# GoogleCloudPlatform/plspm-python

Measured on AMD Instinct MI355X. Metric: bootstrap replicates/sec (6-LV satisfaction model, N=10k), higher is better.
Workload: dtype f64

## Files before the change

plspm-python_amd/csrc/kernels_gram_i8.h:

```cpp
#pragma once
#include <type_traits>
#include "wave_ops.h"

typedef int i32x4 __attribute__((ext_vector_type(4)));
#define I8_SLACK_KB 6
#ifndef I8_DEFAULT_VAR
#define I8_DEFAULT_VAR 3
#endif

__global__ void __launch_bounds__(256) zs_max_kernel(const double* __restrict__ Xa, long N, int PA, int C, const int* __restrict__ pair_p, const int* __restrict__ pair_q,
                                                      int npair, int RB, unsigned long long* __restrict__ pair_max) {
    extern __shared__ __attribute__((aligned(16))) unsigned char smem_raw[];
    double* tile = reinterpret_cast<double*>(smem_raw);
    const int pitch = C | 1;
    const long r0 = (long)blockIdx.x * RB;
    const int nr = (int)min((long)RB, N - r0);
    for (int e = threadIdx.x; e < RB * C; e += 256) {
        const int r = e / C, c = e - r * C;
        tile[r * pitch + c] = (r < nr) ? Xa[(r0 + r) * PA + c] : 0.0;
    }
    __syncthreads();
    for (int j = threadIdx.x; j < npair; j += 256) {
        const int p = pair_p[j], q = pair_q[j];
        double mx = 0.0;
// ... 84 lines not shown
#pragma unroll
            for (int s = 0; s < S; ++s) {
                const int d = (int)((v + 128) & 255) - 128;
                v = (v - d) >> 8;
                dig[s][t] = (unsigned char)(d & 255);
            }
        }
    }
#pragma unroll
    for (int s = 0; s < S; ++s) {
        uint4 w;
        unsigned u[4];
#pragma unroll
        for (int c = 0; c < 4; ++c) u[c] = (unsigned)dig[s][4 * c] | ((unsigned)dig[s][4 * c + 1] << 8) | ((unsigned)dig[s][4 * c + 2] << 16) | ((unsigned)dig[s][4 * c + 3] << 24);
        w.x = u[0]; w.y = u[1]; w.z = u[2]; w.w = u[3];
        if (shape == 16) Zs[((long)kb * NT + (long)pgw * S + s) * 64 + sub * 16 + r] = w;
        else Zs[((long)kb * NT + ((long)pgw * S + s) * 2 + (sub >> 1)) * 64 + (sub & 1) * 32 + r] = w;
    }
}

#define I8_HIST_KB 1024
#define I8_HIST_KB_BYTES 2048
template <bool BYTES>
__global__ void __launch_bounds__(1024) resample_i8_kernel(int N, int KB, int MT, int shape, const int* __restrict__ idx, uint64_t seed, int64_t rep0, uint4* __restrict__ Cd,
                                                           int* __restrict__ err) {
    extern __shared__ __attribute__((aligned(16))) unsigned char smem_raw[];
    unsigned* hist = reinterpret_cast<unsigned*>(smem_raw);
    const int tid = threadIdx.x, nthr = blockDim.x;
    const long b = blockIdx.x;
    constexpr int WKB = BYTES ? I8_HIST_KB_BYTES : I8_HIST_KB;
    const int kb0 = (int)blockIdx.y * WKB, KBw = min(WKB, KB - kb0);
    const unsigned r0 = (unsigned)kb0 * 64u, rspan = (unsigned)KBw * 64u;
    const int nwords = KBw * (BYTES ? 16 : 32);
    auto count = [&](unsigned w) {
        if (BYTES) atomicAdd(&hist[w >> 2], 1u << (8u * (w & 3u)));
        else atomicAdd(&hist[w >> 1], (w & 1u) ? 0x10000u : 1u);
    };
    for (int i = tid; i < nwords; i += nthr) hist[i] = 0u;
    __syncthreads();
    if (idx) {
        const int* my = idx + b * (long)N;
        for (int i = tid; i < N; i += nthr) {
            const int r = my[i];
            if ((unsigned)r < (unsigned)N) { const unsigned w = (unsigned)r - r0; if (w < rspan) count(w); }
            else if (blockIdx.y == 0) atomicOr(err, 1);
        }
    } else {
        const uint64_t rep = (uint64_t)(rep0 + b);
        const int nq = (N + 3) >> 2;
        for (int q = tid; q < nq; q += nthr) {
            const u32x4 u = resample_quad(seed, rep, (uint32_t)q);
#pragma unroll
            for (int j = 0; j < 4; ++j)
                if (4 * q + j < N) { const unsigned w = to_index(u.v[j], (uint32_t)N) - r0; if (w < rspan) count(w); }
        }
    }
    __syncthreads();
    const int mt = (int)(b >> 4), r = (int)(b & 15);
    const uint4* h4 = reinterpret_cast<const uint4*>(hist);
    bool over = false;
    for (int c = tid; c < KBw * 4; c += nthr) {
        uint4 out;
        if (BYTES) {
            out = h4[c];
            over |= ((out.x | out.y | out.z | out.w) & 0x80808080u) != 0u;
        } else {
            const uint4 lo = h4[2 * c], hi = h4[2 * c + 1];
            const unsigned w[8] = {lo.x, lo.y, lo.z, lo.w, hi.x, hi.y, hi.z, hi.w};
            unsigned o[4];
#pragma unroll
            for (int k = 0; k < 4; ++k) {
                const unsigned a = w[2 * k], bb = w[2 * k + 1];
                over |= ((a | bb) & 0xff80ff80u) != 0u;
                o[k] = (a & 0xffu) | ((a >> 8) & 0xff00u) | ((bb & 0xffu) << 16) | ((bb << 8) & 0xff000000u);
            }
            out.x = o[0]; out.y = o[1]; out.z = o[2]; out.w = o[3];
        }
        const int kb = kb0 + (c >> 2), g = c & 3;
        if (shape == 16) Cd[((long)kb * MT + mt) * 64 + g * 16 + r] = out;
        else Cd[((long)kb * MT + (b >> 5) * 2 + (g >> 1)) * 64 + (g & 1) * 32 + (int)(b & 31)] = out;
    }
    if (over) atomicOr(err, 2);
}

#define I8_HIST_KB_NIB 4096
__device__ __forceinline__ unsigned nib_spread16(unsigned t) {
    t = (t | (t << 8)) & 0x00ff00ffu;
    return (t | (t << 4)) & 0x0f0f0f0fu;
}
__global__ void __launch_bounds__(1024) resample_i8_nib_kernel(int N, int KB, int MT, uint64_t seed, int64_t rep0, uint4* __restrict__ Cd, int* __restrict__ err, int force_slow) {
    extern __shared__ __attribute__((aligned(16))) unsigned char smem_raw[];
    unsigned* hist = reinterpret_cast<unsigned*>(smem_raw);
    __shared__ unsigned tot[2];
    const int tid = threadIdx.x, nthr = blockDim.x;
    const long b = blockIdx.x;
    const int kb0 = (int)blockIdx.y * I8_HIST_KB_NIB, KBw = min(I8_HIST_KB_NIB, KB - kb0);
    const unsigned r0 = (unsigned)kb0 * 64u, rspan = (unsigned)KBw * 64u;
    const int nwords = KBw * 8;
    const uint64_t rep = (uint64_t)(rep0 + b);
    const int nq = (N + 3) >> 2;
    const int mt = (int)(b >> 4), r = (int)(b & 15);
    for (int i = tid; i < nwords; i += nthr) hist[i] = 0u;
    if (tid < 2) tot[tid] = 0u;
// ... 560 lines not shown
```

plspm-python_amd/csrc/kernels_gram_i8p.h:

```cpp
#pragma once
#include <type_traits>

template <int S, int MW, int SCHED = 0>
struct GramI8PStep {
    static constexpr int NW = 4, NB = 2 * S, NMFMA = MW * NB;
    static constexpr int PERB = (NB + NW - 1) / NW;
    struct Tab { int a[8], d[8], r[16]; bool ok; };
    static constexpr Tab build() {
        Tab t{};
        if (SCHED == 0) {
            for (int i = 0; i < MW; ++i) t.a[i] = i == 0 ? 1 : NB * i + 1;
            for (int i = 0; i < PERB; ++i) t.d[i] = (i * NMFMA) / PERB + 4;
            for (int r = 0; r < NB; ++r) t.r[r] = (r * (NMFMA - 16)) / NB + 2;
            t.ok = true;
        } else if (SCHED == 2) {
            const int V = MW + PERB;
            bool used[128] = {};
            int na = 0, nd = 0;
            for (int k = 0; k < V; ++k) {
                int m = 1 + (k * NMFMA) / V;
                const bool a_ok = na < MW && m >= (na == 0 ? 1 : NB * na + 1);
                if (a_ok) t.a[na++] = m;
                else if (nd < PERB) t.d[nd++] = m;
                else { m = NB * na + 1; while (used[m]) ++m; t.a[na++] = m; }
// ... 35 lines not shown
    static_assert(MW * NB * 4 <= 240, "accumulator tiles must fit the AGPR half");
};

template <int S, int MTW, int VAR = 0>
struct GramI8P {
    static constexpr int NW = 4, NB = 2 * S, RT = NW * MTW;
    static constexpr int PERB = (NB + NW - 1) / NW;
    static constexpr bool BREG = ((VAR >> 4) & 1) != 0;
    static constexpr int SCHED = (VAR >> 5) & 3;
    static constexpr bool PAIRB = ((VAR >> 7) & 1) != 0 && !BREG;
    static constexpr int STAGE_BYTES = NB * 1024, NS = BREG ? 2 : PAIRB ? 5 : 3, AHEAD = BREG ? 2 : PAIRB ? 4 : 3;
    static constexpr size_t LDS_BYTES = (size_t)NS * STAGE_BYTES;
    static constexpr int RTS = RT - NW;
    static constexpr int ABL = VAR & 15;
};

template <int S, int MTW, int VAR = 0, bool SHORTS = false>
__global__ void __launch_bounds__(256) __attribute__((amdgpu_waves_per_eu(1, 1)))
gram_i8p_kernel(const uint4* __restrict__ Cd, const uint4* __restrict__ Zs, int KB, int MT, int NT, int ntx, int nty, const int* __restrict__ pair_dst,
                const double* __restrict__ pair_scale, int npair, long nrep, double* __restrict__ gram, long psize, int nty_short) {
    using G = GramI8P<S, MTW, VAR>;
    constexpr int NB = G::NB, RT = G::RT;
    extern __shared__ __attribute__((aligned(1024))) unsigned char smem_raw[];
    const int tid = threadIdx.x, lane = tid & 63;
    const int wave = __builtin_amdgcn_readfirstlane(tid >> 6);
    const int w = blockIdx.x;
    int slot = w >> 3, rows = nty, rbase = 0;
    bool shortT = false;
    if constexpr (SHORTS) {
        const int ntall = nty - nty_short, tper = (ntx * ntall + 7) >> 3;
        if (slot >= tper) { slot -= tper; rows = nty_short; rbase = ntall; shortT = true; }
        else rows = ntall;
    }
    const int total = ntx * rows, per = (total + 7) >> 3;
    const int gidx = (w & 7) * per + slot;
    if (slot >= per || gidx >= total) return;
    const int srow = 4 * ntx;
    const int sr = __builtin_amdgcn_readfirstlane(gidx / srow), rem = gidx - sr * srow;
    const int nr = min(4, rows - 4 * sr);
    const int tx = __builtin_amdgcn_readfirstlane(rem / nr), tyl = 4 * sr + (rem - tx * nr);
    const int ct0 = shortT ? rbase * RT + tyl * G::RTS : tyl * RT;

    const unsigned lds0 = (unsigned)(size_t)((__attribute__((address_space(3))) unsigned char*)smem_raw);
    const unsigned voff = (unsigned)lane * 16u;
    const long binc = (long)NT * 1024, ainc = (long)MT * 1024;

// ... 388 lines not shown
```

plspm-python_amd/csrc/model.h:

```cpp
#pragma once
#include <hip/hip_runtime.h>

#include <cstdint>
#include <string>
#include <utility>
#include <vector>

#include "../../include/plspm_hip_test.h"

inline thread_local std::string g_create_error;

hipError_t plspm_dmalloc(void** p, size_t bytes);
void plspm_dfree(void* p);
hipError_t plspm_hmalloc(void** p, size_t bytes);
void plspm_hfree(void* p);
hipError_t plspm_stream_acquire(hipStream_t* s);
void plspm_stream_release(hipStream_t s);

struct PermSpec;
struct StratSpec;
struct CvSpec;
struct JackSpec;

struct ProfSlot { std::vector<std::pair<hipEvent_t, hipEvent_t>> ev, pool; double total_ms = 0.0; int64_t launches = 0; };

struct plspm_model {
    int device = 0;
    hipStream_t stream = nullptr;
    bool owns_stream = true;
    int P = 0, L = 0, PA = 0, T = 0, scheme = 0, scaled = 1, max_iter = 100, kmax = 0, n_eff = 0, n_chol = 0;
    double tol = 1e-6;
// ... 34 lines not shown
    Buf gram2;
    plspm_model* stage2 = nullptr;
    plspm_model* stage1 = nullptr;
    std::vector<int> lv_first, col2_lv1, col2_p1, hcol, hidx;
    std::vector<int> lv_cols;
    int* d_lv_cols = nullptr;
    int *d_lv_first = nullptr, *d_col2_lv1 = nullptr, *d_col2_p1 = nullptr, *d_hcol = nullptr, *d_hidx = nullptr;
    Buf pseudo;
    Buf dcnt, ctable, Xt;
    long dcnt_stride = 0;
    bool Xt_valid = false, dcnt_ready = false;
    int nmx_K = 0, nmx_raw = 0;
    double *d_Xk = nullptr, *d_Mk = nullptr;
    int* d_rowid = nullptr;
    int* h_flag = nullptr;
    hipEvent_t ev_flag = nullptr;
    void* h_stage = nullptr;
    size_t h_stage_cap = 0;
    Buf scores;
    Buf xa, up_raw, up_ci, up_partial;
    int64_t rows_B = 0;
    bool err_clean = false;
    struct Tune { int wide_nw = 4, fit_chunks = 0, conv_pass = 0, conv_gy = 0, nm_threads = 0, solver_threads = 128, scores_tile = 0, gram_lds_kb = 0;
                  int gram_path = 0, i8_slices = 0, i8_min_batch = 1, i8_waves = 8, i8_rt = 0, i8_short = -1, i8_cus = 0, upload_direct = 0, i8_dma = 0, i8_variant = -1, solver_rows = 1, solver_wave = 1, solver_quad = 1, nm_counts8 = 1, nm_fast_lds = 1, nm_k16 = 1, nm_codes = 1, i8_ind = 1, i8_shape = 16, resample_aux = 0, i8_sched = 0, i8_priv = 1, boot_chunks = 0, boot_ratio = 60, boot_align = 0, i8_persist = 0, i8_min_slices = 0, i8_nostore = 0, nm_wave = 1, nm_live = 1, nm_mfma = 1, nm_direct16 = 1, i8_nibbles = 1, nm_wave16 = 1, nm_verify_rows = 0, nm_bound_shift = 0, wide_ring = 4, nm_subset = 4, nm_cat_one = 1, nm_cpl = 0, nm_c10 = 1, nm_vlong = 1, strat_rows = 0, boot_pass = 0; } tune;
    Buf zs, cd, cd1, err2, pair_tab, pair_scale, zs_stat, codes, ind8, tab8, scl8, pp_ctl;
    Buf sk_partial, sk_flags;
    unsigned sk_epoch = 0;
    int cu_count = 0;
    hipStream_t aux = nullptr;
    hipEvent_t ev_counts[2] = {nullptr, nullptr}, ev_cdfree[2] = {nullptr, nullptr};
    bool cdfree_set[2] = {false, false};
    int cd_slot = 0;
    bool zs_valid = false;
    bool zs_stats_ready = false;
    int zs_stats_S = 0;
    void* h_zstat = nullptr;
    size_t h_zstat_cap = 0;
    hipEvent_t ev_zstat = nullptr;
    int zs_S = 0, zs_KB = 0, zs_NT = 0, zs_npair = 0, zs_npg = 0;
    int zs_floor = 0;
    bool zs_ind = false;
    double zs_ratio = 0.0;
    Buf perm_thr, perm_member, perm_io;
    Buf strat_rows, strat_draws, strat_io, strat_u;
    std::vector<uint8_t> strat_member;
    Buf cv_fold, cv_thr, cv_idx, cv_off, cv_mom, cv_coef, cv_io, cv_pred, cv_tab;
    int64_t cv_reps = 0; int cv_k = 0;
    Buf jack_rows, jack_status, jack_iters, jack_io;
    int64_t jack_G = 0;
    bool assess_on = false;
    Buf assess_rows, assess_fit;
    int64_t assess_B = 0;
    bool micom_on = false;
    Buf micom_rows, micom_pool, micom_io;
    int64_t micom_B = 0;
// ... 126 lines not shown
```

plspm-python_amd/csrc/plspm_gram_i8.hip:

```cpp
#include "host_internal.h"

#include "philox.h"
#include "wave_ops.h"
#include "kernels_gram_i8.h"
#include "kernels_gram_i8p.h"

static constexpr size_t kZsBudget = (size_t)24 << 30;
static int cu_count_of(plspm_model* m) {
    if (!m->cu_count) {
        int n = 0;
        if (hipDeviceGetAttribute(&n, hipDeviceAttributeMultiprocessorCount, m->device) == hipSuccess) m->cu_count = n;
    }
    return m->cu_count;
}

bool nm_counts8_possible(const plspm_model* m) {
    return m->nonmetric && m->tune.nm_counts8 != 0 && m->tune.resample_aux == 0 && !m->aux && m->tune.i8_shape == 16 && m->nmx_K == 0 &&
           nm_dense_lds(plan_shape(m), m->tune.conv_pass, nullptr) != 0 && (!m->stage2 || nm_dense_lds(plan_shape(m->stage2), m->stage2->tune.conv_pass, nullptr) != 0);
}
bool gram_i8_closed(const plspm_model* m, int slices) {
    if (m->stage1 || m->N >= (1 << 24) || m->N < 2) return true;
    if (m->nonmetric && m->N > 65535 && !nm_counts8_possible(m)) return true;
    const size_t zs_bytes = (size_t)(i8_kblocks(m->N) + I8_SLACK_KB) * (size_t)(((i8_pairs(m) + 31) / 32) * 2 * (slices ? slices : 7)) * 1024;
    return zs_bytes > kZsBudget;
}
int choose_gram_path(const plspm_model* m, int64_t B) {
    if (m->tune.gram_path == 1 || gram_i8_closed(m, m->tune.i8_slices)) return 1;
    return (m->tune.gram_path == 2 || B >= m->tune.i8_min_batch) ? 2 : 1;
}

static int choose_slices(plspm_model* m, const unsigned long long* h, long npair, int* S_out, int floor) {
    double worst = 1e300;
    unsigned long long any = 0ull;
    for (long j = 0; j < npair; ++j) any |= h[2 * npair + j];
    for (long j = 0; j < npair; ++j) {
        const unsigned long long mb = h[j];
        if (mb == 0) continue;
        const int ef = (int)((mb >> 52) & 0x7ffull);
        if (ef < 64 || ef >= 0x7ff) { worst = 0.0; break; }
        double zmax;
        memcpy(&zmax, &mb, sizeof(double));
// ... 184 lines not shown
        if (!priv) wide20 = m->mix_wide;
        nty_tall = m->mix_tall; nty_short = m->mix_short;
    } else if (wide20 || priv) {
        const long ct = (nb + 15) / 16;
        if (m->tune.i8_short > 0 && (priv || (m->tune.i8_waves == 8 && var20 && m->tune.i8_dma != 2))) nty_short = (int)std::min<long>(m->tune.i8_short, (ct + RTshort - 1) / RTshort);
        nty_tall = (int)std::max(0L, (ct - (long)RTshort * nty_short + RTtall - 1) / RTtall);
    }
    const bool rows2 = wide20 || priv;
    const bool narrow = wide20 || (!priv && m->tune.i8_rt == 8 && m->tune.i8_shape == 16 && m->tune.i8_waves == 4 && m->tune.i8_sched == 0 && m->tune.i8_variant < 0 && S == 7);
    const int RTg = rows2 ? RTtall : narrow ? 8 : 16;
    const bool ind = m->zs_ind && m->tune.i8_sched == 0 && m->tune.i8_variant < 0;
    const int nty = rows2 ? nty_tall + nty_short : (int)((nb + 16 * RTg - 1) / (16 * RTg)), MT = rows2 ? nty_tall * RTtall + nty_short * RTshort : nty * RTg, ntx = ind ? m->zs_npg / 14 : m->zs_npg / 2;
    const bool hist_byte = KB > I8_HIST_KB && !d_idx;
    const bool hist_nib = hist_byte && m->tune.i8_nibbles != 0 && m->tune.i8_shape == 16;
    const int hist_kb = hist_nib ? I8_HIST_KB_NIB : (hist_byte ? I8_HIST_KB_BYTES : I8_HIST_KB);
    const size_t hist_bytes = (size_t)std::min(KB, hist_kb) * (hist_nib ? 8 : (hist_byte ? 16 : 32)) * sizeof(unsigned);
    const unsigned hist_windows = (unsigned)((KB + hist_kb - 1) / hist_kb);
    int rc;
    if ((rc = allow_lds(m, hist_nib ? (const void*)resample_i8_nib_kernel : (hist_byte ? (const void*)resample_i8_kernel<true> : (const void*)resample_i8_kernel<false>), hist_bytes))) return rc;
    const auto resample_k = hist_byte ? resample_i8_kernel<true> : resample_i8_kernel<false>;
    const int nib_slow = m->tune.i8_nibbles == 2 ? 1 : 0;
    m->last_i8_nibbles = hist_nib ? 1 : 0;
    const unsigned resample_threads = (unsigned)std::min(1024, std::max(256, 256 * (int)(8 / std::max<size_t>(1, (160 * 1024) / std::max<size_t>(1, hist_bytes)))));
    if (m->tune.resample_aux && !m->aux) {
        int lo = 0, hi = 0;
        HIPCHK(m, hipDeviceGetStreamPriorityRange(&lo, &hi));
        HIPCHK(m, hipStreamCreateWithPriority(&m->aux, hipStreamNonBlocking, m->tune.resample_aux == 2 ? 0 : (m->tune.resample_aux == 3 ? hi : lo)));
        for (int k = 0; k < 2; ++k) {
            HIPCHK(m, hipEventCreateWithFlags(&m->ev_counts[k], hipEventDisableTiming));
            HIPCHK(m, hipEventCreateWithFlags(&m->ev_cdfree[k], hipEventDisableTiming));
        }
        if ((rc = ensure(m, m->err2, sizeof(int)))) return rc;
        HIPCHK(m, hipMemsetAsync(m->err2.p, 0, sizeof(int), m->aux));
    }
    const int slot = m->aux ? (m->cd_slot ^= 1) : 0;
    plspm_model::Buf& cd = slot ? m->cd1 : m->cd;
    const size_t cd_bytes = (size_t)MT * 16 * ((size_t)KB + I8_SLACK_KB) * 64;
    if (cd_bytes > cd.cap) { if (m->aux) HIPCHK(m, hipStreamSynchronize(m->aux)); if ((rc = ensure(m, cd, cd_bytes))) return rc; m->cdfree_set[slot] = false; }
    if (!d_idx && !brings_counts(call) && m->aux) {
        if (m->cdfree_set[slot]) HIPCHK(m, hipStreamWaitEvent(m->aux, m->ev_cdfree[slot], 0));
        {
            ProfScope ps(m, PLSPM_K_RESAMPLE, m->aux);
            if (hist_nib) hipLaunchKernelGGL(resample_i8_nib_kernel, dim3((unsigned)nb, hist_windows), dim3(resample_threads), hist_bytes, m->aux, (int)m->N, KB, MT, seed, rep0, (uint4*)cd.p, (int*)m->err2.p, nib_slow);
            else
            hipLaunchKernelGGL(resample_k, dim3((unsigned)nb, hist_windows), dim3(resample_threads), hist_bytes, m->aux, (int)m->N, KB, MT, m->tune.i8_shape, d_idx, seed, rep0, (uint4*)cd.p, (int*)m->err2.p);
        }
        HIPCHK(m, hipEventRecord(m->ev_counts[slot], m->aux));
        HIPCHK(m, hipStreamWaitEvent(m->stream, m->ev_counts[slot], 0));
    } else {
        if (m->aux && m->cdfree_set[slot]) HIPCHK(m, hipStreamWaitEvent(m->stream, m->ev_cdfree[slot], 0));
        ProfScope ps(m, PLSPM_K_RESAMPLE);
        rc = 0;
        switch (call.kind) {
            case BatchCall::PERMUTATION: rc = launch_perm_counts(m, *call.perm, nb, rep0, MT, KB, cd.p); break;
            case BatchCall::STRATIFIED: rc = launch_strat_counts(m, *call.strat, nb, rep0, MT, KB, cd.p); break;
            case BatchCall::CROSS_VALIDATION: rc = launch_cv_counts(m, *call.cv, nb, rep0, MT, KB, cd.p); break;
            case BatchCall::JACKKNIFE: rc = launch_jack_counts(m, *call.jack, nb, rep0, MT, KB, cd.p); break;
            case BatchCall::PLAIN:
                if (hist_nib) hipLaunchKernelGGL(resample_i8_nib_kernel, dim3((unsigned)nb, hist_windows), dim3(resample_threads), hist_bytes, m->stream, (int)m->N, KB, MT, seed, rep0, (uint4*)cd.p, (int*)m->err.p, nib_slow);
                else hipLaunchKernelGGL(resample_k, dim3((unsigned)nb, hist_windows), dim3(resample_threads), hist_bytes, m->stream, (int)m->N, KB, MT, m->tune.i8_shape, d_idx, seed, rep0, (uint4*)cd.p, (int*)m->err.p);
                break;
        }
        if (rc) return rc;
    }
    if (d_idx) {
        int* h_err = (int*)m->h_flag + 9;
        HIPCHK(m, hipMemcpyAsync(h_err, m->err.p, sizeof(int), hipMemcpyDeviceToHost, m->stream));
        HIPCHK(m, hipStreamSynchronize(m->stream));
        if (*h_err & 2) {
            const int keep = *h_err & 1;
            HIPCHK(m, hipMemcpyAsync(m->err.p, &keep, sizeof(int), hipMemcpyHostToDevice, m->stream));
            HIPCHK(m, hipStreamSynchronize(m->stream));
            *fallback = true;
            return 0;
        }
    }
    if (counts && m->tune.i8_shape == 16) { *counts = cd.p; *counts_MT = MT; }
    const int total = ntx * nty, per = rows2 ? (ntx * nty_tall + 7) / 8 + (ntx * nty_short + 7) / 8 : (total + 7) / 8;
    const bool to16 = out16 && wrote16 && ind && m->tune.i8_shape == 16;
    const int* d_dst = (const int*)m->pair_tab.p + (to16 ? 6 : (dense ? 4 : 3)) * (size_t)m->zs_npair;
    const int* d_dst2 = nullptr;
    const long out_stride = to16 ? (long)(m->Pg + 1) * ((m->Pg + 1 + 7) & ~7) : (dense ? cov_doubles(m->Pg) : packed_size(m->T));
    if (to16) { out = reinterpret_cast<double*>(out16); *wrote16 = true; }
    const bool sk = m->tune.i8_sched == 1 && m->tune.i8_shape == 16 && m->tune.i8_variant < 0 && S >= 5 && S <= 7;
    int sk_grid = 0;
    if (sk) {
        if (!cu_count_of(m)) return fail(m, PLSPM_E_STATE, "hipDeviceGetAttribute(multiprocessor count) failed");
        sk_grid = std::max(8, (m->cu_count / 8) * 8);
        const size_t slot_bytes = (size_t)32 * S * 1024;
        if ((size_t)sk_grid * slot_bytes > m->sk_partial.cap && (rc = ensure(m, m->sk_partial, (size_t)sk_grid * slot_bytes))) return rc;
        if (!m->sk_flags.p) {
            if ((rc = ensure(m, m->sk_flags, (size_t)2048 * 8 * sizeof(unsigned)))) return rc;
            HIPCHK(m, hipMemsetAsync(m->sk_flags.p, 0, (size_t)2048 * 8 * sizeof(unsigned), m->stream));
            m->sk_epoch = 0;
        }
    }
    const bool dma_fits = (uint64_t)(KB + I8_SLACK_KB) * (uint64_t)std::max(MT, NT) * 1024ull < (1ull << 32);
    const bool dma_buffer = !priv && m->tune.i8_dma != 1 && dma_fits && m->tune.i8_shape == 16 && !sk && (!narrow || (wide20 && m->tune.i8_waves == 4)) && m->tune.i8_variant < 0;
    m->last_i8_dma = dma_buffer ? 2 : 1;
    m->last_i8_rt = RTg;
    m->last_i8_short = rows2 ? nty_short : 0;
    m->last_i8_priv = priv ? 1 : 0;
    m->last_i8_mt = MT;
    ProfScope ps(m, PLSPM_K_GRAM);
#ifdef PLSPM_I8_EXPERIMENTS
#define I8_FOUR_WAVES (m->tune.i8_waves == 4)
#else
#define I8_FOUR_WAVES false
#endif
#define GI8SK(SS, WW)                                                                                                                        \
    {                                                                                                                                        \
        const size_t lds_bytes = GramI8<SS, WW, I8_DEFAULT_VAR, 16>::LDS_BYTES;                                                              \
        if ((rc = allow_lds(m, (const void*)gram_i8_sk_kernel<SS, WW>, lds_bytes))) return rc;                                               \
        hipLaunchKernelGGL((gram_i8_sk_kernel<SS, WW>), dim3((unsigned)sk_grid), dim3(128 * WW), lds_bytes, m->stream, (const uint4*)cd.p,    \
                           (const uint4*)m->zs.p, KB, MT, NT, ntx, nty, d_dst, (const double*)m->pair_scale.p, m->zs_npair, (long)nb, out, out_stride, \
                           (i32x4*)m->sk_partial.p, (unsigned*)m->sk_flags.p, ++m->sk_epoch, (int*)m->err.p);                                \
    }
#define GI8P(SS, MM, VV)                                                                                                                     \
    {                                                                                                                                        \
        const size_t lds_bytes = GramI8P<SS, MM, VV>::LDS_BYTES;                                                                             \
        auto kfn = nty_short ? gram_i8p_kernel<SS, MM, VV, true> : gram_i8p_kernel<SS, MM, VV, false>;                                       \
        if ((rc = allow_lds(m, (const void*)kfn, lds_bytes))) return rc;                                                                     \
        hipLaunchKernelGGL(kfn, dim3((unsigned)(8 * per)), dim3(256), lds_bytes, m->stream, (const uint4*)cd.p,                               \
                           (const uint4*)m->zs.p, KB, MT, NT, ntx, nty, d_dst, (const double*)m->pair_scale.p, m->zs_npair, nb_launch, out, out_stride, nty_short); \
    }
#define GI8PP(SS, MM)                                                                                                                        \
// ... 94 lines not shown
#endif
#ifdef PLSPM_I8_EXPERIMENTS
    if (wide20 && m->tune.i8_waves == 4) { if (dma_buffer) GI8RT20(2, I8_DEFAULT_VAR + 800) else GI8RT20(2, I8_DEFAULT_VAR) } else
    if (narrow && !wide20) GI8RT(8) else
    if (m->tune.i8_shape == 32 && S >= 5) {
        switch (S) { case 5: GI8VS(5, 2, I8_DEFAULT_VAR, 32) break; case 6: GI8VS(6, 2, I8_DEFAULT_VAR, 32) break; case 7: GI8VS(7, 2, I8_DEFAULT_VAR, 32) break; default: GI8VS(8, 2, I8_DEFAULT_VAR, 32) break; }
    } else
    if (m->tune.i8_waves == 4) {
        if (dma_buffer) { switch (S) { case 1: GI8B(1, 2) break; case 2: GI8B(2, 2) break; case 3: GI8B(3, 2) break; case 4: GI8B(4, 2) break; case 5: GI8B(5, 2) break; case 6: GI8B(6, 2) break; case 7: GI8B(7, 2) break; default: GI8B(8, 2) break; } }
        else { switch (S) { case 1: GI8(1, 2) break; case 2: GI8(2, 2) break; case 3: GI8(3, 2) break; case 4: GI8(4, 2) break; case 5: GI8(5, 2) break; case 6: GI8(6, 2) break; case 7: GI8(7, 2) break; default: GI8(8, 2) break; } }
    } else
#endif
    if (wide20) GI8RT20(4, I8_DEFAULT_VAR) else
    if (dma_buffer) {
        switch (S) { case 1: GI8B(1, 4) break; case 2: GI8B(2, 4) break; case 3: GI8B(3, 4) break; case 4: GI8B(4, 4) break; case 5: GI8B(5, 4) break; case 6: GI8B(6, 4) break; case 7: GI8B(7, 4) break; default: GI8B(8, 4) break; }
    } else {
        switch (S) { case 1: GI8(1, 4) break; case 2: GI8(2, 4) break; case 3: GI8(3, 4) break; case 4: GI8(4, 4) break; case 5: GI8(5, 4) break; case 6: GI8(6, 4) break; case 7: GI8(7, 4) break; default: GI8(8, 4) break; }
    }
#undef GI8V
#undef GI8VS
#undef GI8
#undef GI8B
    HIPCHK(m, hipGetLastError());
    if (m->aux) { HIPCHK(m, hipEventRecord(m->ev_cdfree[slot], m->stream)); m->cdfree_set[slot] = true; }
    return 0;
}

int64_t plspm_detail_round_units_peek(const plspm_model* m) {
    if (!m || !m->d_Xa || m->nonmetric || m->n_ind || !m->zs_valid || !m->cu_count || choose_gram_path(m, (int64_t)1 << 20) != 2) return 64;
    const int S = m->zs_S;
    if ((S != 6 && S != 7) || m->zs_ind || m->tune.i8_priv == 0) return 64;
    const int cus = std::max(8, m->tune.i8_cus > 0 ? std::min(m->tune.i8_cus, m->cu_count) : m->cu_count);
    const int ntx = std::max(1, m->zs_npg / 2), tall = (S == 6 ? 20 : 16) * 16;
    return (int64_t)std::max(1, cus / ntx) * tall;
}

int64_t plspm_detail_round_units(plspm_model* m) {
    if (!m || !m->d_Xa || m->nonmetric || m->n_ind || choose_gram_path(m, (int64_t)1 << 20) != 2) return 64;
    if (hipSetDevice(m->device) != hipSuccess || prepare_zs(m)) return 64;
    if (!cu_count_of(m)) return 64;
    return plspm_detail_round_units_peek(m);
}

extern "C" {

int plspm_bootstrap_prepare(plspm_model_t* m) {
    if (!m) return PLSPM_E_ARG;
    if (!m->d_Xa || m->N < 2) return fail(m, PLSPM_E_STATE, "plspm_bootstrap_prepare: no data uploaded");
// ... 15 lines not shown
```

plspm-python_amd/csrc/plspm_hip.hip:

```cpp
#include "host_internal.h"

#include "philox.h"
#include "kernels_upload.h"

namespace {
struct MemPool {
    std::mutex mu;
    std::multimap<size_t, void*> idle[17];
    std::unordered_map<void*, std::pair<int, size_t>> live;
    size_t idle_bytes[17] = {};
};
MemPool& pool() { static MemPool* p = new MemPool(); return *p; }
constexpr size_t kPoolKeepPerDevice = (size_t)8 << 30, kPoolMaxBlock = (size_t)1 << 30, kPoolKeepHost = (size_t)1 << 30;
size_t size_class(size_t bytes) {
    if (bytes <= 2048) return (bytes + 255) & ~(size_t)255;
    int lg = 63 - __builtin_clzll((unsigned long long)bytes);
    const size_t step = (size_t)1 << (lg - 3);
    return (bytes + step - 1) & ~(step - 1);
}
hipError_t pool_get(int idx, size_t bytes, void** out) {
    const size_t want = size_class(std::max<size_t>(bytes, 1));
    MemPool& P = pool();
    {
        std::lock_guard<std::mutex> lock(P.mu);
// ... 248 lines not shown
    if (m->stream) hipStreamSynchronize(m->stream);
    prof_collect(m);
    void* ptrs[] = {m->d_shift, m->xa.p, m->up_raw.p, m->up_ci.p, m->up_partial.p, m->scores.p,
                    m->d_mv_base2, m->d_lmv2_off, m->gSm.p, m->d_ind_of, m->gram2.p, m->pseudo.p, m->d_Xk, m->d_Mk, m->d_rowid, m->dcnt.p, m->ctable.p, m->Xt.p,
                    m->ent.p, m->nent.p, m->gram.p, m->gram_partial.p, m->rows.p, m->status.p, m->iters.p, m->gS.p, m->gsmall.p,
                    m->fitout.p, m->idx.p, m->err.p, m->ghist.p, m->nmstate.p, m->nmpartial.p, m->nmactive.p, m->nmlist.p, m->gK16.p, m->sum_buf.p, m->cols.p,
                    m->nmw_maps.p, m->nmw_ints.p, m->nmw_vsum.p, m->zs.p, m->cd.p, m->cd1.p, m->codes.p, m->ind8.p, m->tab8.p, m->scl8.p, m->err2.p, m->pp_ctl.p, m->sk_partial.p, m->sk_flags.p, m->pair_tab.p, m->pair_scale.p, m->zs_stat.p,
                    m->perm_thr.p, m->perm_member.p, m->perm_io.p, m->strat_rows.p, m->strat_draws.p, m->strat_io.p, m->strat_u.p,
                    m->cv_fold.p, m->cv_thr.p, m->cv_idx.p, m->cv_off.p, m->cv_mom.p, m->cv_coef.p, m->cv_io.p, m->cv_pred.p, m->cv_tab.p,
                    m->jack_rows.p, m->jack_status.p, m->jack_iters.p, m->jack_io.p, m->assess_rows.p, m->assess_fit.p, m->micom_rows.p, m->micom_pool.p, m->micom_io.p};
    for (void* p : ptrs) if (p) plspm_dfree(p);
    for (void* p : m->blobs) if (p) plspm_dfree(p);
    if (m->h_stage) plspm_hfree(m->h_stage);
    if (m->h_pin) plspm_hfree(m->h_pin);
    for (int k = 0; k < 2; ++k) if (m->ev_pin[k]) hipEventDestroy(m->ev_pin[k]);
    for (auto& e : m->ev_part) if (e) hipEventDestroy(e);
    if (m->dl) { hipStreamSynchronize(m->dl); plspm_stream_release(m->dl); }
    if (m->ev_pin_async) hipEventDestroy(m->ev_pin_async);
    for (int k = 0; k < PLSPM_K_COUNT; ++k) for (auto& pr : m->prof[k].pool) { hipEventDestroy(pr.first); hipEventDestroy(pr.second); }
    if (m->h_flag) plspm_hfree(m->h_flag);
    if (m->h_zstat) plspm_hfree(m->h_zstat);
    if (m->ev_zstat) hipEventDestroy(m->ev_zstat);
    if (m->ev_flag) hipEventDestroy(m->ev_flag);
    for (int k = 0; k < 2; ++k) { if (m->ev_counts[k]) hipEventDestroy(m->ev_counts[k]); if (m->ev_cdfree[k]) hipEventDestroy(m->ev_cdfree[k]); }
    if (m->aux) hipStreamDestroy(m->aux);
    if (m->stream && m->owns_stream) plspm_stream_release(m->stream);
    delete m;
}

int32_t plspm_effect_pairs(const plspm_model_t* m, int32_t* from, int32_t* to) {
    if (!m) return 0;
    for (int e = 0; e < m->n_eff; ++e) { if (from) from[e] = m->eff_from[e]; if (to) to[e] = m->eff_to[e]; }
    return m->n_eff;
}
int32_t plspm_row_width(const plspm_model_t* m) {
    if (!m) return 0;
    if (m->stage2) m = m->stage2;
    return 2 * (m->categorical ? m->Pm : m->P) + m->L + 2 * m->n_eff;
}
int32_t plspm_row_stride(const plspm_model_t* m) { return m ? plspm_row_width(m) + 2 : 0; }

int plspm_upload(plspm_model_t* m, const double* X, int64_t N, int32_t src_cols, int32_t layout, const int32_t* col_index) {
    if (!m) return PLSPM_E_ARG;
    if (!X || N < 2 || src_cols < 1 || (layout != 0 && layout != 1)) return fail(m, PLSPM_E_ARG, "plspm_upload: bad arguments");
    if (N > 0x7fffffffLL - 64) return fail(m, PLSPM_E_LIMIT, "plspm_upload: N must fit in int32");
    const int Pg = m->Pg;
    std::vector<int> ci(Pg);
// ... 109 lines not shown
    else if (k == "nm_mfma") { if (value < 0 || value > 1) return bad(); m->tune.nm_mfma = value; }
    else if (k == "nm_direct16") { if (value < 0 || value > 1) return bad(); m->tune.nm_direct16 = value; }
    else if (k == "i8_nibbles") { if (value < 0 || value > 2) return bad(); m->tune.i8_nibbles = value; }
    else if (k == "strat_rows") { if (value < 0 || value > 2) return bad(); m->tune.strat_rows = value; }
    else if (k == "nm_wave") { if (value < 0 || value > 1) return bad(); m->tune.nm_wave = value; }
    else if (k == "i8_ind") { if (value < 0 || value > 1) return bad(); if (value != m->tune.i8_ind) m->zs_valid = false; m->tune.i8_ind = value; }
    else if (k == "upload_direct") { if (value < 0 || value > 1) return bad(); m->tune.upload_direct = value; }
    else if (k == "i8_short_rows") { if (value < -1 || value > 4096) return bad(); m->tune.i8_short = value; }
    else if (k == "i8_cus") { if (value != 0 && (value < 8 || value > 4096)) return bad(); m->tune.i8_cus = value; }
    else if (k == "i8_rt") { if (value != 0 && value != 16 && value != 8 && value != 20) return bad(); if (value == 8 && !experiments) return exp_only(); m->tune.i8_rt = value; }
    else if (k == "solver_rows") { if (value != 0 && value != 1) return bad(); m->tune.solver_rows = value; }
    else if (k == "solver_wave") { if (value < 0 || value > 3) return bad(); m->tune.solver_wave = value; }
    else if (k == "solver_quad") { if (value != 0 && value != 1) return bad(); m->tune.solver_quad = value; }
    else if (k == "nm_live") { if (value != 0 && value != 1) return bad(); m->tune.nm_live = value; }
    else if (k == "nm_wave16") { if (value != 0 && value != 1) return bad(); m->tune.nm_wave16 = value; }
    else if (k == "nm_subset") { if (value < 0 || value > 100) return bad(); m->tune.nm_subset = value; }
    else if (k == "nm_cpl") { if (value != 0 && value != 8 && value != 6) return bad(); m->tune.nm_cpl = value; }
    else if (k == "nm_c10") { if (value != 0 && value != 1) return bad(); m->tune.nm_c10 = value; }
    else if (k == "nm_vlong") { if (value != 0 && value != 1) return bad(); m->tune.nm_vlong = value; }
    else if (k == "nm_cat_one") { if (value != 0 && value != 1) return bad(); m->tune.nm_cat_one = value; }
    else if (k == "nm_bound_shift") { if (value < 0 || value > 200) return bad(); m->tune.nm_bound_shift = value; }
    else if (k == "nm_verify_rows") { if (value < 0 || value > 100) return bad(); m->tune.nm_verify_rows = value; }
    else if (k == "nm_counts8") { if (value != 0 && value != 1) return bad(); m->tune.nm_counts8 = value; }
    else if (k == "resample_aux") { if (value < 0 || value > 3) return bad(); if (value && !experiments) return exp_only(); m->tune.resample_aux = value; }
    else if (k == "i8_sched") { if (value != 0 && value != 1) return bad(); if (value && !experiments) return exp_only(); m->tune.i8_sched = value; }
    else if (k == "i8_priv") { if (value < 0 || value > 1) return bad(); m->tune.i8_priv = value; }
    else if (k == "i8_persist") { if (value < 0 || value > 1) return bad(); m->tune.i8_persist = value; }
    else if (k == "i8_nostore") { if (value < 0 || value > 1) return bad(); if (value && !experiments) return exp_only(); m->tune.i8_nostore = value; }
    else if (k == "i8_shape") { if (value != 16 && value != 32) return bad(); if (value != 16 && !experiments) return exp_only(); if (value != m->tune.i8_shape) m->zs_valid = false; m->tune.i8_shape = value; }
    else if (k == "i8_variant") { if (value < -1 || value > 899) return bad(); if (value >= 0 && !experiments) return exp_only(); m->tune.i8_variant = value; }
    else if (k == "i8_dma") { if (value < 0 || value > 2) return bad(); m->tune.i8_dma = value; }
    else if (k == "conv_gy") { if (value < 0 || value > 65535) return bad(); m->tune.conv_gy = value; }
    else if (k == "boot_chunks") { if (value < 0 || value > kBootChunksMax) return bad(); m->tune.boot_chunks = value; }
    else if (k == "boot_ratio") { if (value < 10 || value > 100) return bad(); m->tune.boot_ratio = value; }
    else if (k == "boot_align") { if (value < 0 || value > (1 << 20)) return bad(); m->tune.boot_align = value; }
    else if (k == "boot_pass") { if (value < 0 || value > (1 << 30) || (value & 255)) return bad(); m->tune.boot_pass = value; }
    else return fail(m, PLSPM_E_ARG, "plspm_model_set_option: unknown option '" + k + "'");
    if (m->group) plspm_detail_group_plan_changed(m->group);
    return 0;
}

int plspm_model_get_option(const plspm_model_t* m, const char* key, int32_t* value) {
    if (!m || !key || !value) return PLSPM_E_ARG;
    const std::string k(key);
    if (k == "solver_threads") *value = m->tune.solver_threads;
    else if (k == "nm_threads") *value = m->tune.nm_threads;
    else if (k == "fit_chunks") *value = m->tune.fit_chunks;
// ... 31 lines not shown
    else if (k == "upload_direct") *value = m->tune.upload_direct;
    else if (k == "i8_dma") *value = m->tune.i8_dma;
    else if (k == "last_i8_dma") *value = m->last_i8_dma;
    else if (k == "solver_rows") *value = m->tune.solver_rows;
    else if (k == "solver_wave") *value = m->tune.solver_wave;
    else if (k == "solver_quad") *value = m->tune.solver_quad;
    else if (k == "nm_live") *value = m->tune.nm_live;
    else if (k == "nm_wave16") *value = m->tune.nm_wave16;
    else if (k == "nm_verify_rows") *value = m->tune.nm_verify_rows;
    else if (k == "nm_bound_shift") *value = m->tune.nm_bound_shift;
    else if (k == "nm_subset") *value = m->tune.nm_subset;
    else if (k == "nm_cat_one") *value = m->tune.nm_cat_one;
    else if (k == "nm_cpl") *value = m->tune.nm_cpl;
    else if (k == "nm_c10") *value = m->tune.nm_c10;
    else if (k == "nm_vlong") *value = m->tune.nm_vlong;
    else if (k == "last_nm_one") *value = m->last_nm_one;
    else if (k == "last_nm_exact") *value = m->last_nm_exact;
    else if (k == "last_nm_wave16") *value = m->last_nm_wave16;
    else if (k == "last_nm_flagged") *value = m->last_nm_flagged;
    else if (k == "last_nm_replayed") *value = m->last_nm_replayed;
    else if (k == "nm_counts8") *value = m->tune.nm_counts8;
    else if (k == "last_solver") *value = m->last_solver;
    else if (k == "resample_aux") *value = m->tune.resample_aux;
    else if (k == "i8_sched") *value = m->tune.i8_sched;
    else if (k == "i8_priv") *value = m->tune.i8_priv;
    else if (k == "last_i8_priv") *value = m->last_i8_priv;
    else if (k == "i8_persist") *value = m->tune.i8_persist;
    else if (k == "nm_wave") *value = m->tune.nm_wave;
    else if (k == "last_nm_wave") *value = m->last_nm_wave;
    else if (k == "i8_min_slices") *value = m->tune.i8_min_slices;
    else if (k == "last_i8_persist") *value = m->last_i8_persist;
    else if (k == "i8_shape") *value = m->tune.i8_shape;
    else if (k == "boot_chunks") *value = m->tune.boot_chunks;
    else if (k == "boot_ratio") *value = m->tune.boot_ratio;
    else if (k == "boot_align") *value = m->tune.boot_align;
    else if (k == "boot_round_units") *value = (int32_t)plspm_detail_round_units_peek(m);
    else if (k == "boot_pass") *value = m->tune.boot_pass;
    else if (k == "last_boot_passes") *value = m->last_boot_passes;
    else if (k == "last_gram_path") *value = m->last_gram_path;
    else if (k == "last_micom_layout") *value = m->last_micom_layout;
    else if (k == "build_experiments") {
#ifdef PLSPM_I8_EXPERIMENTS
        *value = 1;
#else
        *value = 0;
#endif
// ... 301 lines not shown
```

Measured before the change: 10.71 million.

## Refactor aux-stream resample ring, pack histogram with perm, raise gram priority

Moves the double-buffered count-slot event logic for running resample draws on an auxiliary stream into a CountsRing helper, adds a GO event, and gates aux use on plain metric calls. Aux use still defaults to off. Separately, the 16-bit histogram packing now uses a byte-permute builtin, the output address computation is unified across shapes, the resample kernel is capped to 8 VGPRs, and the i8 gram kernel raises its wave priority. The VGPR cap risks register spills, and the priority bump may starve concurrent kernels.

After: 10.62 million. About the same (-0.8%).

```diff
diff --git a/plspm-python_amd/csrc/counts_ring.h b/plspm-python_amd/csrc/counts_ring.h
--- /dev/null
+++ b/plspm-python_amd/csrc/counts_ring.h
@@ -0,0 +1,43 @@
+#pragma once
+
+struct CountsRing {
+    enum Stream { MAIN = 0, AUX = 1 };
+    enum Event { COUNTS0 = 0, COUNTS1 = 1, FREE0 = 2, FREE1 = 3, GO = 4, N_EVENTS = 5 };
+    int slot = 0;
+    bool free_set[2] = {false, false};
+    bool go_set = false;
+
+    int next_slot(bool has_aux) { return has_aux ? (slot ^= 1) : 0; }
+    void grown(int s) { free_set[s] = false; }
+    template <class Wait>
+    int before_draws(int s, bool on_aux, bool has_aux, Wait&& wait) {
+        int rc = 0;
+        if (on_aux) {
+            if (free_set[s] && (rc = wait(AUX, FREE0 + s))) return rc;
+            if (go_set && (rc = wait(AUX, GO))) return rc;
+        } else if (has_aux && free_set[s]) {
+            rc = wait(MAIN, FREE0 + s);
+        }
+        return rc;
+    }
+    template <class Record, class Wait>
+    int after_draws(int s, bool on_aux, Record&& record, Wait&& wait) {
+        if (!on_aux) return 0;
+        if (int rc = record(AUX, COUNTS0 + s)) return rc;
+        return wait(MAIN, COUNTS0 + s);
+    }
+    template <class Record>
+    int before_gram(bool has_aux, Record&& record) {
+        if (!has_aux) return 0;
+        if (int rc = record(MAIN, GO)) return rc;
+        go_set = true;
+        return 0;
+    }
+    template <class Record>
+    int after_gram(int s, bool has_aux, Record&& record) {
+        if (!has_aux) return 0;
+        if (int rc = record(MAIN, FREE0 + s)) return rc;
+        free_set[s] = true;
+        return 0;
+    }
+};
diff --git a/plspm-python_amd/csrc/kernels_gram_i8.h b/plspm-python_amd/csrc/kernels_gram_i8.h
--- a/plspm-python_amd/csrc/kernels_gram_i8.h
+++ b/plspm-python_amd/csrc/kernels_gram_i8.h
@@ -130,7 +130,7 @@
 #define I8_HIST_KB 1024
 #define I8_HIST_KB_BYTES 2048
 template <bool BYTES>
-__global__ void __launch_bounds__(1024) resample_i8_kernel(int N, int KB, int MT, int shape, const int* __restrict__ idx, uint64_t seed, int64_t rep0, uint4* __restrict__ Cd,
+__global__ void __launch_bounds__(1024) __attribute__((amdgpu_num_vgpr(8))) resample_i8_kernel(int N, int KB, int MT, int shape, const int* __restrict__ idx, uint64_t seed, int64_t rep0, uint4* __restrict__ Cd,
                                                            int* __restrict__ err) {
     extern __shared__ __attribute__((aligned(16))) unsigned char smem_raw[];
     unsigned* hist = reinterpret_cast<unsigned*>(smem_raw);
@@ -142,7 +142,7 @@
     const int nwords = KBw * (BYTES ? 16 : 32);
     auto count = [&](unsigned w) {
         if (BYTES) atomicAdd(&hist[w >> 2], 1u << (8u * (w & 3u)));
-        else atomicAdd(&hist[w >> 1], (w & 1u) ? 0x10000u : 1u);
+        else atomicAdd(&hist[w >> 1], 1u << ((w & 1u) << 4));
     };
     for (int i = tid; i < nwords; i += nthr) hist[i] = 0u;
     __syncthreads();
@@ -164,7 +164,8 @@
         }
     }
     __syncthreads();
-    const int mt = (int)(b >> 4), r = (int)(b & 15);
+    const bool s16 = shape == 16;
+    const int col0 = s16 ? (int)(b >> 4) : (int)(b >> 5) * 2, row0 = s16 ? (int)(b & 15) : (int)(b & 31), gsh = s16 ? 2 : 1, gmask = s16 ? 3 : 1;
     const uint4* h4 = reinterpret_cast<const uint4*>(hist);
     bool over = false;
     for (int c = tid; c < KBw * 4; c += nthr) {
@@ -173,20 +174,19 @@
             out = h4[c];
             over |= ((out.x | out.y | out.z | out.w) & 0x80808080u) != 0u;
         } else {
-            const uint4 lo = h4[2 * c], hi = h4[2 * c + 1];
-            const unsigned w[8] = {lo.x, lo.y, lo.z, lo.w, hi.x, hi.y, hi.z, hi.w};
-            unsigned o[4];
-#pragma unroll
-            for (int k = 0; k < 4; ++k) {
-                const unsigned a = w[2 * k], bb = w[2 * k + 1];
-                over |= ((a | bb) & 0xff80ff80u) != 0u;
-                o[k] = (a & 0xffu) | ((a >> 8) & 0xff00u) | ((bb & 0xffu) << 16) | ((bb << 8) & 0xff000000u);
-            }
-            out.x = o[0]; out.y = o[1]; out.z = o[2]; out.w = o[3];
+            unsigned all = 0u;
+            auto pack = [&](unsigned a, unsigned bb) {
+                all |= a | bb;
+                return __builtin_amdgcn_perm(bb, a, 0x06040200u);
+            };
+            const uint4 lo = h4[2 * c];
+            out.x = pack(lo.x, lo.y); out.y = pack(lo.z, lo.w);
+            const uint4 hi = h4[2 * c + 1];
+            out.z = pack(hi.x, hi.y); out.w = pack(hi.z, hi.w);
+            over |= (all & 0xff80ff80u) != 0u;
         }
         const int kb = kb0 + (c >> 2), g = c & 3;
-        if (shape == 16) Cd[((long)kb * MT + mt) * 64 + g * 16 + r] = out;
-        else Cd[((long)kb * MT + (b >> 5) * 2 + (g >> 1)) * 64 + (g & 1) * 32 + (int)(b & 31)] = out;
+        Cd[((long)kb * MT + col0 + (g >> gsh)) * 64 + ((g & gmask) << (6 - gsh)) + row0] = out;
     }
     if (over) atomicOr(err, 2);
 }
diff --git a/plspm-python_amd/csrc/kernels_gram_i8p.h b/plspm-python_amd/csrc/kernels_gram_i8p.h
--- a/plspm-python_amd/csrc/kernels_gram_i8p.h
+++ b/plspm-python_amd/csrc/kernels_gram_i8p.h
@@ -81,6 +81,7 @@
     using G = GramI8P<S, MTW, VAR>;
     constexpr int NB = G::NB, RT = G::RT;
     extern __shared__ __attribute__((aligned(1024))) unsigned char smem_raw[];
+    __builtin_amdgcn_s_setprio(3);
     const int tid = threadIdx.x, lane = tid & 63;
     const int wave = __builtin_amdgcn_readfirstlane(tid >> 6);
     const int w = blockIdx.x;
diff --git a/plspm-python_amd/csrc/model.h b/plspm-python_amd/csrc/model.h
--- a/plspm-python_amd/csrc/model.h
+++ b/plspm-python_amd/csrc/model.h
@@ -7,6 +7,11 @@
 #include <vector>
 
 #include "../../include/plspm_hip_test.h"
+#include "counts_ring.h"
+
+#ifndef PLSPM_RESAMPLE_AUX_DEFAULT
+#define PLSPM_RESAMPLE_AUX_DEFAULT 0
+#endif
 
 inline thread_local std::string g_create_error;
 
@@ -87,15 +92,16 @@
     int64_t rows_B = 0;
     bool err_clean = false;
     struct Tune { int wide_nw = 4, fit_chunks = 0, conv_pass = 0, conv_gy = 0, nm_threads = 0, solver_threads = 128, scores_tile = 0, gram_lds_kb = 0;
-                  int gram_path = 0, i8_slices = 0, i8_min_batch = 1, i8_waves = 8, i8_rt = 0, i8_short = -1, i8_cus = 0, upload_direct = 0, i8_dma = 0, i8_variant = -1, solver_rows = 1, solver_wave = 1, solver_quad = 1, nm_counts8 = 1, nm_fast_lds = 1, nm_k16 = 1, nm_codes = 1, i8_ind = 1, i8_shape = 16, resample_aux = 0, i8_sched = 0, i8_priv = 1, boot_chunks = 0, boot_ratio = 60, boot_align = 0, i8_persist = 0, i8_min_slices = 0, i8_nostore = 0, nm_wave = 1, nm_live = 1, nm_mfma = 1, nm_direct16 = 1, i8_nibbles = 1, nm_wave16 = 1, nm_verify_rows = 0, nm_bound_shift = 0, wide_ring = 4, nm_subset = 4, nm_cat_one = 1, nm_cpl = 0, nm_c10 = 1, nm_vlong = 1, strat_rows = 0, boot_pass = 0; } tune;
+                  int gram_path = 0, i8_slices = 0, i8_min_batch = 1, i8_waves = 8, i8_rt = 0, i8_short = -1, i8_cus = 0, upload_direct = 0, i8_dma = 0, i8_variant = -1, solver_rows = 1, solver_wave = 1, solver_quad = 1, nm_counts8 = 1, nm_fast_lds = 1, nm_k16 = 1, nm_codes = 1, i8_ind = 1, i8_shape = 16, resample_aux = PLSPM_RESAMPLE_AUX_DEFAULT, i8_sched = 0, i8_priv = 1, boot_chunks = 0, boot_ratio = 60, boot_align = 0, i8_persist = 0, i8_min_slices = 0, i8_nostore = 0, nm_wave = 1, nm_live = 1, nm_mfma = 1, nm_direct16 = 1, i8_nibbles = 1, nm_wave16 = 1, nm_verify_rows = 0, nm_bound_shift = 0, wide_ring = 4, nm_subset = 4, nm_cat_one = 1, nm_cpl = 0, nm_c10 = 1, nm_vlong = 1, strat_rows = 0, boot_pass = 0; } tune;
     Buf zs, cd, cd1, err2, pair_tab, pair_scale, zs_stat, codes, ind8, tab8, scl8, pp_ctl;
     Buf sk_partial, sk_flags;
     unsigned sk_epoch = 0;
     int cu_count = 0;
     hipStream_t aux = nullptr;
-    hipEvent_t ev_counts[2] = {nullptr, nullptr}, ev_cdfree[2] = {nullptr, nullptr};
-    bool cdfree_set[2] = {false, false};
-    int cd_slot = 0;
+    hipEvent_t ev_ring[CountsRing::N_EVENTS] = {nullptr, nullptr, nullptr, nullptr, nullptr};
+    CountsRing ring;
+    int last_resample_aux = 0;
+    bool aux_explicit = false;
     bool zs_valid = false;
     bool zs_stats_ready = false;
     int zs_stats_S = 0;
diff --git a/plspm-python_amd/csrc/plspm_gram_i8.hip b/plspm-python_amd/csrc/plspm_gram_i8.hip
--- a/plspm-python_amd/csrc/plspm_gram_i8.hip
+++ b/plspm-python_amd/csrc/plspm_gram_i8.hip
@@ -14,9 +14,14 @@
     return m->cu_count;
 }
 
-bool nm_counts8_possible(const plspm_model* m) {
-    return m->nonmetric && m->tune.nm_counts8 != 0 && m->tune.resample_aux == 0 && !m->aux && m->tune.i8_shape == 16 && m->nmx_K == 0 &&
+static bool nm_counts8_wanted(const plspm_model* m) {
+    return m->nonmetric && m->tune.nm_counts8 != 0 && m->tune.i8_shape == 16 && m->nmx_K == 0 &&
            nm_dense_lds(plan_shape(m), m->tune.conv_pass, nullptr) != 0 && (!m->stage2 || nm_dense_lds(plan_shape(m->stage2), m->stage2->tune.conv_pass, nullptr) != 0);
+}
+bool nm_counts8_possible(const plspm_model* m) { return !m->aux && nm_counts8_wanted(m); }
+static bool aux_draws_allowed(const plspm_model* m, const BatchCall& call) {
+    if (m->tune.resample_aux == 0 || call.kind != BatchCall::PLAIN || call.d_idx || nm_counts8_wanted(m)) return false;
+    return m->aux_explicit || plain_metric(m);
 }
 bool gram_i8_closed(const plspm_model* m, int slices) {
     if (m->stage1 || m->N >= (1 << 24) || m->N < 2) return true;
@@ -247,33 +252,33 @@
     const int nib_slow = m->tune.i8_nibbles == 2 ? 1 : 0;
     m->last_i8_nibbles = hist_nib ? 1 : 0;
     const unsigned resample_threads = (unsigned)std::min(1024, std::max(256, 256 * (int)(8 / std::max<size_t>(1, (160 * 1024) / std::max<size_t>(1, hist_bytes)))));
-    if (m->tune.resample_aux && !m->aux) {
+    const bool want_aux = aux_draws_allowed(m, call);
+    if (want_aux && !m->aux) {
         int lo = 0, hi = 0;
         HIPCHK(m, hipDeviceGetStreamPriorityRange(&lo, &hi));
         HIPCHK(m, hipStreamCreateWithPriority(&m->aux, hipStreamNonBlocking, m->tune.resample_aux == 2 ? 0 : (m->tune.resample_aux == 3 ? hi : lo)));
-        for (int k = 0; k < 2; ++k) {
-            HIPCHK(m, hipEventCreateWithFlags(&m->ev_counts[k], hipEventDisableTiming));
-            HIPCHK(m, hipEventCreateWithFlags(&m->ev_cdfree[k], hipEventDisableTiming));
-        }
+        for (auto& e : m->ev_ring) HIPCHK(m, hipEventCreateWithFlags(&e, hipEventDisableTiming));
         if ((rc = ensure(m, m->err2, sizeof(int)))) return rc;
         HIPCHK(m, hipMemsetAsync(m->err2.p, 0, sizeof(int), m->aux));
     }
-    const int slot = m->aux ? (m->cd_slot ^= 1) : 0;
+    const bool has_aux = m->aux != nullptr, on_aux = want_aux && has_aux;
+    auto ring_wait = [&](int stream, int event) { HIPCHK(m, hipStreamWaitEvent(stream == CountsRing::AUX ? m->aux : m->stream, m->ev_ring[event], 0)); return 0; };
+    auto ring_record = [&](int stream, int event) { HIPCHK(m, hipEventRecord(m->ev_ring[event], stream == CountsRing::AUX ? m->aux : m->stream)); return 0; };
+    const int slot = m->ring.next_slot(has_aux);
     plspm_model::Buf& cd = slot ? m->cd1 : m->cd;
     const size_t cd_bytes = (size_t)MT * 16 * ((size_t)KB + I8_SLACK_KB) * 64;
-    if (cd_bytes > cd.cap) { if (m->aux) HIPCHK(m, hipStreamSynchronize(m->aux)); if ((rc = ensure(m, cd, cd_bytes))) return rc; m->cdfree_set[slot] = false; }
-    if (!d_idx && !brings_counts(call) && m->aux) {
-        if (m->cdfree_set[slot]) HIPCHK(m, hipStreamWaitEvent(m->aux, m->ev_cdfree[slot], 0));
-        {
-            ProfScope ps(m, PLSPM_K_RESAMPLE, m->aux);
-            if (hist_nib) hipLaunchKernelGGL(resample_i8_nib_kernel, dim3((unsigned)nb, hist_windows), dim3(resample_threads), hist_bytes, m->aux, (int)m->N, KB, MT, seed, rep0, (uint4*)cd.p, (int*)m->err2.p, nib_slow);
-            else
-            hipLaunchKernelGGL(resample_k, dim3((unsigned)nb, hist_windows), dim3(resample_threads), hist_bytes, m->aux, (int)m->N, KB, MT, m->tune.i8_shape, d_idx, seed, rep0, (uint4*)cd.p, (int*)m->err2.p);
-        }
-        HIPCHK(m, hipEventRecord(m->ev_counts[slot], m->aux));
-        HIPCHK(m, hipStreamWaitEvent(m->stream, m->ev_counts[slot], 0));
+    if (cd_bytes > cd.cap) {
+        if (has_aux) { HIPCHK(m, hipStreamSynchronize(m->aux)); HIPCHK(m, hipStreamSynchronize(m->stream)); }
+        if ((rc = ensure(m, cd, cd_bytes))) return rc;
+        m->ring.grown(slot);
+    }
+    m->last_resample_aux = on_aux ? 1 : 0;
+    if ((rc = m->ring.before_draws(slot, on_aux, has_aux, ring_wait))) return rc;
+    if (on_aux) {
+        ProfScope ps(m, PLSPM_K_RESAMPLE, m->aux);
+        if (hist_nib) hipLaunchKernelGGL(resample_i8_nib_kernel, dim3((unsigned)nb, hist_windows), dim3(resample_threads), hist_bytes, m->aux, (int)m->N, KB, MT, seed, rep0, (uint4*)cd.p, (int*)m->err2.p, nib_slow);
+        else hipLaunchKernelGGL(resample_k, dim3((unsigned)nb, hist_windows), dim3(resample_threads), hist_bytes, m->aux, (int)m->N, KB, MT, m->tune.i8_shape, d_idx, seed, rep0, (uint4*)cd.p, (int*)m->err2.p);
     } else {
-        if (m->aux && m->cdfree_set[slot]) HIPCHK(m, hipStreamWaitEvent(m->stream, m->ev_cdfree[slot], 0));
         ProfScope ps(m, PLSPM_K_RESAMPLE);
         rc = 0;
         switch (call.kind) {
@@ -288,6 +293,7 @@
         }
         if (rc) return rc;
     }
+    if ((rc = m->ring.after_draws(slot, on_aux, ring_record, ring_wait))) return rc;
     if (d_idx) {
         int* h_err = (int*)m->h_flag + 9;
         HIPCHK(m, hipMemcpyAsync(h_err, m->err.p, sizeof(int), hipMemcpyDeviceToHost, m->stream));
@@ -327,6 +333,7 @@
     m->last_i8_short = rows2 ? nty_short : 0;
     m->last_i8_priv = priv ? 1 : 0;
     m->last_i8_mt = MT;
+    if ((rc = m->ring.before_gram(has_aux, ring_record))) return rc;
     ProfScope ps(m, PLSPM_K_GRAM);
 #ifdef PLSPM_I8_EXPERIMENTS
 #define I8_FOUR_WAVES (m->tune.i8_waves == 4)
@@ -467,8 +474,7 @@
 #undef GI8
 #undef GI8B
     HIPCHK(m, hipGetLastError());
-    if (m->aux) { HIPCHK(m, hipEventRecord(m->ev_cdfree[slot], m->stream)); m->cdfree_set[slot] = true; }
-    return 0;
+    return m->ring.after_gram(slot, has_aux, ring_record);
 }
 
 int64_t plspm_detail_round_units_peek(const plspm_model* m) {
diff --git a/plspm-python_amd/csrc/plspm_hip.hip b/plspm-python_amd/csrc/plspm_hip.hip
--- a/plspm-python_amd/csrc/plspm_hip.hip
+++ b/plspm-python_amd/csrc/plspm_hip.hip
@@ -294,7 +294,7 @@
     if (m->h_zstat) plspm_hfree(m->h_zstat);
     if (m->ev_zstat) hipEventDestroy(m->ev_zstat);
     if (m->ev_flag) hipEventDestroy(m->ev_flag);
-    for (int k = 0; k < 2; ++k) { if (m->ev_counts[k]) hipEventDestroy(m->ev_counts[k]); if (m->ev_cdfree[k]) hipEventDestroy(m->ev_cdfree[k]); }
+    for (auto& e : m->ev_ring) if (e) hipEventDestroy(e);
     if (m->aux) hipStreamDestroy(m->aux);
     if (m->stream && m->owns_stream) plspm_stream_release(m->stream);
     delete m;
@@ -450,7 +450,7 @@
     else if (k == "nm_bound_shift") { if (value < 0 || value > 200) return bad(); m->tune.nm_bound_shift = value; }
     else if (k == "nm_verify_rows") { if (value < 0 || value > 100) return bad(); m->tune.nm_verify_rows = value; }
     else if (k == "nm_counts8") { if (value != 0 && value != 1) return bad(); m->tune.nm_counts8 = value; }
-    else if (k == "resample_aux") { if (value < 0 || value > 3) return bad(); if (value && !experiments) return exp_only(); m->tune.resample_aux = value; }
+    else if (k == "resample_aux") { if (value < 0 || value > 3) return bad(); if (value > 1 && !experiments) return exp_only(); m->tune.resample_aux = value; m->aux_explicit = true; }
     else if (k == "i8_sched") { if (value != 0 && value != 1) return bad(); if (value && !experiments) return exp_only(); m->tune.i8_sched = value; }
     else if (k == "i8_priv") { if (value < 0 || value > 1) return bad(); m->tune.i8_priv = value; }
     else if (k == "i8_persist") { if (value < 0 || value > 1) return bad(); m->tune.i8_persist = value; }
@@ -528,6 +528,7 @@
     else if (k == "nm_counts8") *value = m->tune.nm_counts8;
     else if (k == "last_solver") *value = m->last_solver;
     else if (k == "resample_aux") *value = m->tune.resample_aux;
+    else if (k == "last_resample_aux") *value = m->last_resample_aux;
     else if (k == "i8_sched") *value = m->tune.i8_sched;
     else if (k == "i8_priv") *value = m->tune.i8_priv;
     else if (k == "last_i8_priv") *value = m->last_i8_priv;
```
